# balisujohn/tortoise.cpp

Measured on AMD Instinct MI355X. Metric: audio-seconds/sec end-to-end (AR+diffusion+vocoder), 16 cands x 80 steps, higher is better.
Workload: dtype f16 MFMA inputs / f32 accumulate (diffusion, vocoder convs); f32 weights, f16 KV (AR)

## Files before the change

tortoise.cpp_amd/csrc/api.cpp:

```cpp
#include "common.h"
#include <sched.h>
#include <cctype>
#include <cstddef>
#include <cmath>
#include <algorithm>
#include <chrono>
#include <fstream>
#include <new>

using namespace tts;

hipEvent_t tts::prof_event(tts_ctx *c) {
  if (!c->ev_pool.empty()) { hipEvent_t e = c->ev_pool.back(); c->ev_pool.pop_back(); return e; }
  hipEvent_t e = nullptr;
  (void)hipEventCreate(&e);
  return e;
}

template <class F>
static int guarded(tts_ctx *c, F body) {
  try {
    return body();
  } catch (const std::bad_alloc &) {
    return fail(c, TTS_ERR_LIMIT, "out of host memory");
// ... 130 lines not shown
static void ar_control_store(int which, double value, SamplerParams &sp, int &scope) {
  switch (which) {
  case 0: sp.temp = (float)value; break;
  case 1: sp.top_k = (int)value; break;
  case 2: sp.top_p = (float)value; break;
  case 3: sp.penalty = (float)value; break;
  case 4: scope = (int)value; break;
  case 5: sp.typ_mass = (float)value; break;
  }
}

int tts_set_option(tts_ctx *c, const char *key, double value) {
  if (!c || !key) return TTS_ERR_ARG;
  std::string k(key);
  if (k == "gn_eps") c->gn_eps = (float)value;
  else if (k == "ggml_lut") c->ggml_lut = value != 0;
  else if (k.rfind("prof_only:", 0) == 0) {
    if (value != 0) c->prof_filter.push_back(k.substr(10));
    else c->prof_filter.clear();
  }
  else if (k == "device_topk") c->device_topk = value != 0;
  else if (k == "sampler_threads") {
    if (c->sampler_pool) { sampler_pool_free(c->sampler_pool); c->sampler_pool = nullptr; }
    c->sampler_threads = value < 0 ? -1 : (int)value;
  }
  else if (k == "share_uncond") c->share_uncond = value != 0;
  else if (k == "prof_stride") c->prof_stride = value < 1 ? 1 : (int)value;
  else if (k == "diff_graph") c->diff_graph = value != 0;
  else if (k == "dec_f32_mfma") c->dec_f32_mfma = value != 0;
  else if (k == "attn_f32") c->attn_f32 = value != 0;
  else if (k == "attn_proj_f16") c->attn_proj_f16 = value != 0;
  else if (k == "proj_dual_b") c->proj_dual_b = value != 0;
  else if (k == "gemm_wreg") c->gemm_wreg = value == 1 ? tts_ctx::GEMM_WREG_ALL : value == 2 ? 1 : value == 3 ? 2 : value == 4 ? 4 : 0;
  else if (k == "lc_attn_f32") c->lc_attn_f32 = value != 0;
  else if (k == "latency_mode") c->latency_mode = value != 0;
  else if (k == "fp16_check") c->fp16_check = value != 0;
  else if (k == "rng_fast_normal") c->rng_fast_normal = value != 0;
  else if (k == "noise_pipeline") c->noise_pipeline = value != 0;
  else if (k == "load_device_pack") c->load_device_pack = value != 0;
  else if (k == "load_threads") c->load_threads = value < 0 ? 0 : value > 64 ? 64 : (int)value;
  else if (k == "attn_q64") c->attn_q64 = value < 0 ? 0 : value > 2 ? 2 : (int)value;
  else if (k == "hoist_integrator") c->hoist_integrator = value < 0 ? 0 : (int)value;
  else if (k == "attn_f32_drop") c->attn_f32_drop = (int)value & 7;
  else if (k == "ar_weights") {
    if (value != 0 && value != 1 && value != 2) return fail(c, TTS_ERR_ARG, "ar_weights: 0 (f32), 1 (fp16) or 2 (fp8 e4m3)");
    c->ar_weights = (int)value;
  }
  else if (k == "diff_sampler") {
    if (const char *e = diff_control_error(0, value)) return fail(c, TTS_ERR_ARG, "%s", e);
    c->diff_sampler = (int)value;
  }
  else if (k == "ddim_eta") {
    if (const char *e = diff_control_error(1, value)) return fail(c, TTS_ERR_ARG, "%s", e);
    c->ddim_eta = value;
  }
  else if (k == "cond_free_k") {
    if (const char *e = diff_control_error(2, value)) return fail(c, TTS_ERR_ARG, "%s", e);
    c->cond_free_k = (float)value;
  }
  else if (k == "diff_temperature") {
    if (const char *e = diff_control_error(3, value)) return fail(c, TTS_ERR_ARG, "%s", e);
    c->diff_temperature = value;
  }
  else if (k == "cond_free") {
    if (const char *e = diff_control_error(4, value)) return fail(c, TTS_ERR_ARG, "%s", e);
    c->cond_free = (int)value;
// ... 702 lines not shown
```

tortoise.cpp_amd/csrc/common.h:

```cpp
#pragma once
#include "../../include/tortoise_mi355x.h"
#include <hip/hip_runtime.h>
#include <cstdarg>
#include <cstdint>
#include <cstdio>
#include <cstring>
#include <functional>
#include <map>
#include <memory>
#include <random>
#include <algorithm>
#include <atomic>
#include <condition_variable>
#include <mutex>
#include <new>
#include <string>
#include <thread>
#include <vector>

namespace tts {

struct HostTensor {
  std::vector<float> data;
  int64_t ne[4] = {1, 1, 1, 1};
// ... 90 lines not shown
  std::normal_distribution<double> normal_distribution{0.0, 1.0};
  uint32_t seed_value = 0;
  tts::ArState *ar = nullptr;
  tts::DiffState *diff = nullptr;
  tts::VocState *voc = nullptr;
  tts::ClvpState *clvp = nullptr;
  tts::CvvpState *cvvp = nullptr;
  tts::VoiceEncState *venc = nullptr;
  tts::DiffCondEncState *dcond = nullptr;
  tts::HifiganState *hifigan = nullptr;
  tts::AfeState *afe = nullptr;
  tts::Tokenizer *tok = nullptr;
  tts::ArSession *session = nullptr;
  tts::DiffSession *diff_session = nullptr;
  tts::SamplerPool *sampler_pool = nullptr;
  tts::SamplerParams ar_sp;
  int ar_penalty_scope = 0;
  int device_topk = 1;
  int time_mlp_retries = 0;
  int topk_fallbacks = 0;
  int sampler_threads = -1;
  bool share_uncond = true;
  int rng_shard_offset = 0, rng_shard_total = 0;
  std::vector<int32_t> stop_schedule;
  std::vector<int32_t> ar_stopped;
  bool prof_on = false;
  std::vector<std::string> prof_filter;
  int prof_stride = 1;
  int ar_weights = 0;
  int dec_f32_mfma = 0;
  int attn_f32 = 0;
  static constexpr int GEMM_WREG_ALL = 7;
  int gemm_wreg = GEMM_WREG_ALL;
  int proj_dual_b = 1;
  int attn_f32_drop = 0;
  int lc_attn_f32 = 1;
  int attn_proj_f16 = 0;
  int fp16_check = 0;
  int64_t fp16_bad_weights[2] = {0, 0};
  void *fp16_counts = nullptr;
  int rng_fast_normal = 1;
  int noise_pipeline = 1;
  int load_device_pack = 1;
  int load_threads = 0;
  int attn_q64 = 0;
  int hoist_integrator = 1;
  int latency_mode = 0;
  int diff_sampler = 0;
  double ddim_eta = 0;
  float cond_free_k = 2.0f;
  int cond_free = 1;
  double diff_temperature = 1.0;
  int last_diff_rows = -1, last_diff_seqs = 0;
  bool capturing = false;
  int stream_recaptures = 0;
  int hfg_small_m = 0;
  int diff_graph = 1;
  int prof_eager_every = 8;
  std::map<std::string, tts::ProfEntry> prof;
  std::vector<hipEvent_t> ev_pool;
  hipEvent_t ev0 = nullptr, ev1 = nullptr;
};

namespace tts {

int fail(tts_ctx *ctx, int code, const char *fmt, ...);
// ... 313 lines not shown
```

tortoise.cpp_amd/csrc/diffusion.hip:

```cpp
#include "common.h"
#include "gemm_f16.h"
#include <algorithm>
#include <chrono>
#include <cmath>

namespace tts {

static constexpr int C = 1024, NHEAD = 16, XTC = 128 ;
static constexpr int LAT_MAX_ROWS = 2048;
static constexpr int HOIST_MAX_ROWS = 16384;

__device__ __forceinline__ float silu_dev(float x, int lut) {
  if (lut == 1) {
    float xr = __half2float(__float2half_rn(x));
    return __half2float(__float2half_rn(xr / (1.0f + expf(-xr))));
  }
  if (lut == 2) return x / (1.0f + expf(-x));
  return x * __builtin_amdgcn_rcpf(1.0f + __builtin_amdgcn_exp2f(x * -1.44269504088896f));
}

__global__ __launch_bounds__(256) void gn_stats_kernel(const float *__restrict__ x, const int *__restrict__ seq_start,
                                                       const int *__restrict__ seq_len, float eps, float2 *__restrict__ stats) {
  __shared__ float sh[8];
  const int grp = blockIdx.x, s = blockIdx.y, T = seq_len[s];
// ... 1219 lines not shown
  ProfScope ps(ctx, fam, 2.0 * mv * (n_valid ? n_valid : g.N) * (k_valid ? k_valid : g.nseg * g.kseg));
  TTS_HIP(ctx, launch_gemm_f16(g, ctx->stream));
  if (ctx->fp16_check) {
    if (gemm_mode_qkv(g.mode)) {
      CHECK(fp16_check(ctx, g.outH, (size_t)g.M * g.ldh));
      CHECK(fp16_check(ctx, g.outVt, (size_t)(g.N / 3) * g.ldvt));
    } else if (g.mode == GEMM_OUT_F16) CHECK(fp16_check(ctx, g.outH, (size_t)g.M * g.ldh));
  }
  return TTS_OK;
}

static int gemm_wreg_class(const tts_ctx *ctx, int bit) { return (ctx->gemm_wreg & bit) ? 1 : 0; }
static const __half *gemm_wreg_image(const tts_ctx *ctx, int bit, const Layout &lay, int N, const __half *w, const __half *wf) {
  return gemm_wreg_class(ctx, bit) && gemm_auto_th(lay.rows, N) == 8 ? wf : w;
}

static GemmArgs gemm_base(const Layout &lay, const __half *A, int lda, int nseg, int kseg, const __half *W, int N,
                          const float *bias) {
  GemmArgs g{};
  for (int i = 0; i < 3; i++) { g.A[i] = A; g.row_off[i] = 0; }
  if (nseg == 3) { g.row_off[0] = -1; g.row_off[1] = 0; g.row_off[2] = 1; }
  g.nseg = nseg; g.kseg = kseg; g.lda = lda; g.W = W; g.M = lay.rows; g.N = N; g.bias = bias;
  g.row_seq = lay.d_row_seq.as<int>();
  return g;
}

static int gn_stats(tts_ctx *ctx, const Layout &lay, Work &wk, const float *x) {
  ProfScope ps(ctx, "diff_gn_stats");
  gn_stats_kernel<<<dim3(32, lay.ns), 256, 0, ctx->stream>>>(x, lay.d_start.as<int>(), lay.d_len.as<int>(), ctx->gn_eps,
                                                             wk.stats.as<float2>());
  TTS_HIP(ctx, hipGetLastError());
  return TTS_OK;
}
template <int NT, int NJ>
__global__ __launch_bounds__(NT) void gn_reg_kernel(const float *__restrict__ x, const int *__restrict__ seq_start,
                                                    const int *__restrict__ seq_len, int rows_total, int ns, float eps,
                                                    const float *__restrict__ g, const float *__restrict__ b,
                                                    const float *__restrict__ ss, int do_silu, int lut, __half *__restrict__ y,
                                                    const char *__restrict__ pf0, int pf0_lines, const char *__restrict__ pf1, int pf1_lines,
                                                    const int *__restrict__ seq_step, int ss_step_stride) {
  constexpr int NW = NT / 64, SWEEP = NT / 8;
  __shared__ float sh[2][NW];
  __shared__ unsigned pf_sink[NW][64];
  const int bid = blockIdx.y * 32 + blockIdx.x, nbk = ns * 32, item = (bid & 7) * (nbk >> 3) + (bid >> 3);
  const int s = item >> 5, grp = item & 31;
  const int T = seq_len[s], r0 = seq_start[s];
  const int q = threadIdx.x & 7, c = grp * 32 + q * 4, t0 = threadIdx.x >> 3;
  const float *base = x + (size_t)r0 * C + c;
  float4 v[NJ];
#pragma unroll
  for (int j = 0; j < NJ; j++) {
    const int t = t0 + j * SWEEP;
    v[j] = *(const float4 *)(base + (size_t)min(t, T - 1) * C);
  }
  {
    const int gi = (blockIdx.y * 32 + blockIdx.x) * NT + threadIdx.x, tt = 32 * ns * NT;
    unsigned *sink = &pf_sink[__builtin_amdgcn_readfirstlane(threadIdx.x >> 6)][0];
    for (int l = gi; l < pf0_lines; l += tt) __builtin_amdgcn_global_load_lds((gptr_t)(pf0 + (size_t)l * 128), (lptr_t)sink, 4, 0, 0);
    for (int l = gi; l < pf1_lines; l += tt) __builtin_amdgcn_global_load_lds((gptr_t)(pf1 + (size_t)l * 128), (lptr_t)sink, 4, 0, 0);
  }
  const float4 gg = *(const float4 *)(g + c), bb = *(const float4 *)(b + c);
  float sc4[4] = {1.f, 1.f, 1.f, 1.f}, sh4[4] = {0.f, 0.f, 0.f, 0.f};
  if (ss) {
    if (seq_step) ss += (size_t)seq_step[s] * ss_step_stride;
#pragma unroll
    for (int i = 0; i < 4; i++) { sc4[i] = ss[c + i] + 1.0f; sh4[i] = ss[C + c + i]; }
  }
  float sum = 0.f;
#pragma unroll
  for (int j = 0; j < NJ; j++)
    if (t0 + j * SWEEP < T) sum += (v[j].x + v[j].y) + (v[j].z + v[j].w);
#pragma unroll
  for (int o = 32; o > 0; o >>= 1) sum += __shfl_xor(sum, o);
  if ((threadIdx.x & 63) == 0) sh[0][threadIdx.x >> 6] = sum;
  __syncthreads();
  float tot = 0.f;
#pragma unroll
  for (int w = 0; w < NW; w++) tot += sh[0][w];
  const float n = (float)T * 32.f, mean = tot / n;
  float sq = 0.f;
#pragma unroll
  for (int j = 0; j < NJ; j++) {
    v[j].x -= mean; v[j].y -= mean; v[j].z -= mean; v[j].w -= mean;
    if (t0 + j * SWEEP < T) sq += (v[j].x * v[j].x + v[j].y * v[j].y) + (v[j].z * v[j].z + v[j].w * v[j].w);
  }
#pragma unroll
  for (int o = 32; o > 0; o >>= 1) sq += __shfl_xor(sq, o);
  if ((threadIdx.x & 63) == 0) sh[1][threadIdx.x >> 6] = sq;
  __syncthreads();
  float tsq = 0.f;
#pragma unroll
  for (int w = 0; w < NW; w++) tsq += sh[1][w];
  const float rstd = 1.0f / sqrtf(tsq / n + eps);
  const float ge[4] = {gg.x, gg.y, gg.z, gg.w}, be[4] = {bb.x, bb.y, bb.z, bb.w};
  auto apply = [&](auto mode) {
    constexpr int MODE = decltype(mode)::value;
#pragma unroll
    for (int j = 0; j < NJ; j++) {
      const int t = min(t0 + j * SWEEP, T - 1);
      float e[4] = {v[j].x, v[j].y, v[j].z, v[j].w};
#pragma unroll
      for (int i = 0; i < 4; i++) {
        float u = e[i] * rstd;
        u = u * ge[i];
        u = u + be[i];
        u = u * sc4[i];
        u = u + sh4[i];
        if (MODE) u = silu_dev(u, MODE - 1);
        e[i] = u;
      }
      const __half2 p0 = __floats2half2_rn(e[0], e[1]), p1 = __floats2half2_rn(e[2], e[3]);
      uint2 o;
      o.x = *(const unsigned *)&p0;
      o.y = *(const unsigned *)&p1;
      *(uint2 *)(y + (size_t)(r0 + t) * C + c) = o;
    }
  };
  if (!do_silu) apply(std::integral_constant<int, 0>{});
  else if (lut == 0) apply(std::integral_constant<int, 1>{});
  else if (lut == 1) apply(std::integral_constant<int, 2>{});
  else apply(std::integral_constant<int, 3>{});
  const int gend = (s + 1 < ns) ? seq_start[s + 1] : rows_total;
  for (int r = r0 + T + t0; r < gend; r += SWEEP) *(uint2 *)(y + (size_t)r * C + c) = make_uint2(0u, 0u);
  if (s == 0)
    for (int r = t0; r < r0; r += SWEEP) *(uint2 *)(y + (size_t)r * C + c) = make_uint2(0u, 0u);
  if (pf0_lines | pf1_lines) asm volatile("s_waitcnt vmcnt(0)" ::: "memory");
}

static int gn_fused(tts_ctx *ctx, const Layout &lay, const float *x, const float *g, const float *b, const float *ss, int do_silu,
                    __half *y, const void *wa = nullptr, size_t wa_bytes = 0, const void *wb = nullptr, size_t wb_bytes = 0) {
  ProfScope ps(ctx, "diff_gn_fused");
  if (lay.rows > 4096) { wa_bytes = 0; wb_bytes = 0; }
  const int silu_mode = ctx->ggml_lut ? 1 : ctx->attn_f32 ? 2 : 0;
  auto launch = [&](const int *d_start, int s0, int ns, int row0, int rows, int tmax) {
    const float *xp = x + (size_t)row0 * C;
    __half *yp = y + (size_t)row0 * C;
    const int *d_len = lay.d_len.as<int>() + s0, *step = lay.seq_step_ptr() ? lay.seq_step_ptr() + s0 : nullptr;
#define GN_ARGS xp, d_start, d_len, rows, ns, ctx->gn_eps, g, b, ss, do_silu, silu_mode, yp, \
                (const char *)wa, (int)(wa_bytes >> 7), (const char *)wb, (int)(wb_bytes >> 7), step, lay.ss_step_stride
    if (tmax <= 14 * 64) gn_reg_kernel<512, 14><<<dim3(32, ns), 512, 0, ctx->stream>>>(GN_ARGS);
    else if (tmax <= 18 * 128) gn_reg_kernel<1024, 18><<<dim3(32, ns), 1024, 0, ctx->stream>>>(GN_ARGS);
    else gn_fused_kernel<0><<<dim3(32, ns), 256, 0, ctx->stream>>>(xp, d_start, d_len, rows, ns, ctx->gn_eps, g, b, ss,
                                                                  do_silu, silu_mode, yp, step, lay.ss_step_stride);
#undef GN_ARGS
  };
  if (lay.gn_parts.empty()) launch(lay.d_start.as<int>(), 0, lay.ns, 0, lay.rows, lay.max_len());
  else for (const Layout::GnPart &p : lay.gn_parts) launch(lay.d_start_rel.as<int>() + p.s0, p.s0, p.ns, p.row0, p.rows, p.tmax);
  TTS_HIP(ctx, hipGetLastError());
  return TTS_OK;
}

__global__ __launch_bounds__(256) void gn_apply_kernel(const float *__restrict__ x, const int *__restrict__ chunk_seq, const int *__restrict__ seq_start,
                                                       const int *__restrict__ seq_len, const long long *__restrict__ st, int stripe_ll, float eps, const float *__restrict__ g,
                                                       const float *__restrict__ b, const float *__restrict__ ss, int do_silu, int lut, __half *__restrict__ y,
                                                       const char *__restrict__ pf0, int pf0_lines, const char *__restrict__ pf1, int pf1_lines,
                                                       const int *__restrict__ seq_step, int ss_step_stride) {
  __shared__ float2 mr[32];
  __shared__ unsigned pf_sink[4][64];
  const int r0 = blockIdx.x * 4, s = chunk_seq[blockIdx.x >> 1], c = threadIdx.x * 4;
// ... 134 lines not shown
    }
    TTS_HIP(ctx, hipGetLastError());
  }
  CHECK(fp16_check(ctx, wk.ATT16(), (size_t)lay.rows * C));
  if (f32 && (ctx->attn_f32_drop & 4)) TTS_HIP(ctx, hipMemsetAsync(wk.att16_lo.p, 0, (size_t)(wk.rows + 2) * C * 2, ctx->stream));
  DBG_SUM("attn out", wk.ATT16(), (size_t)lay.rows * C * 2);
  if (f32) {
    GemmArgs p = gemm_base(lay, wk.ATT16(), C, 3, C, w.proj_w_split, C, w.proj_b);
    p.A[0] = wk.ATT16(); p.A[1] = wk.att16_lo.as<__half>() + C; p.A[2] = wk.ATT16();
    p.row_off[0] = p.row_off[1] = p.row_off[2] = 0;
    p.custom_w = 1; p.ldw_ = 2 * C; p.w_off_[0] = 0; p.w_off_[1] = 0; p.w_off_[2] = C;
    p.mode = st_out ? GEMM_OUT_F32_SCALED_STATS : GEMM_OUT_F32_SCALED; p.alpha = w.proj_alpha; p.outF = X; p.ldo = C; p.resid = X;
    p.st_out = st_out; p.st_stripe_ll = (int)st->gn_stripe_ll; p.chunk_seq = lay.d_chunk_seq.as<int>();
    return gemm(ctx, "diff_gemm", p, lay, 0, C);
  }
  if (!ctx->attn_proj_f16) {
    GemmArgs p = gemm_base(lay, wk.ATT16(), C, 2, C, w.proj_w_split, C, w.proj_b);
    p.custom_w = 1; p.ldw_ = 2 * C; p.w_off_[0] = 0; p.w_off_[1] = C;
    p.mode = st_out ? GEMM_OUT_F32_SCALED_STATS : GEMM_OUT_F32_SCALED; p.alpha = w.proj_alpha; p.outF = X; p.ldo = C; p.resid = X;
    p.st_out = st_out; p.st_stripe_ll = (int)st->gn_stripe_ll; p.chunk_seq = lay.d_chunk_seq.as<int>();
    p.dual_b = ctx->proj_dual_b;
    CHECK(gemm(ctx, "diff_gemm", p, lay, 0, C));
    DBG_SUM("attn proj", X, (size_t)lay.rows * C * 4);
    return TTS_OK;
  }
  GemmArgs p = gemm_base(lay, wk.ATT16(), C, 1, C, w.proj_w, C, w.proj_b);
  p.mode = st_out ? GEMM_OUT_F32_STATS : GEMM_OUT_F32; p.outF = X; p.ldo = C; p.resid = X;
  p.st_out = st_out; p.st_stripe_ll = (int)st->gn_stripe_ll; p.chunk_seq = lay.d_chunk_seq.as<int>();
  CHECK(gemm(ctx, "diff_gemm", p, lay));
  DBG_SUM("attn proj", X, (size_t)lay.rows * C * 4);
  return TTS_OK;
}

static int res_block(tts_ctx *ctx, DiffState *st, const Layout &lay, Work &wk, float *X, const ResDev &w, const float *ss,
                     const float *Xin = nullptr, const float *Hpre = nullptr, const long long *st_hpre = nullptr) {
  const float *xin = Xin ? Xin : X;
  const bool lat = st->lat && (Hpre ? st_hpre != nullptr : wk.st_x != nullptr);
  const long long *st_h = st_hpre;
  if (!Hpre) {
    long long *slot = lat ? st->new_stats_slot() : nullptr;
    CHECK(res_in_layers(ctx, st, lay, wk, xin, w, wk.H(), lat ? wk.st_x : nullptr, slot));
    Hpre = wk.H();
    st_h = slot;
  }
  DBG_SUM("res.out ss", ss, (size_t)2 * C * 4);
  DBG_SUM("res.out hpre", Hpre, (size_t)lay.rows * C * 4);
  CHECK(gn(ctx, st, lay, Hpre, lat ? st_h : nullptr, w.out_g, w.out_b, ss, 1, wk.A16(), lat ? w.out_w : gemm_wreg_image(ctx, 4, lay, C, w.out_w, w.out_wf), (size_t)3 * C * C * 2));
  DBG_SUM("res.out gn", wk.A16(), (size_t)lay.rows * C * 2);
  GemmArgs c3 = gemm_base(lay, wk.A16(), C, 3, C, w.out_w, C, w.out_bias);
  c3.Wf = w.out_wf; c3.wreg = gemm_wreg_class(ctx, 4);
  long long *st_out = lat ? st->new_stats_slot() : nullptr;
  c3.mode = st_out ? GEMM_OUT_F32_STATS : GEMM_OUT_F32; c3.outF = X; c3.ldo = C; c3.resid = xin;
  c3.st_out = st_out; c3.st_stripe_ll = (int)st->gn_stripe_ll; c3.chunk_seq = lay.d_chunk_seq.as<int>();
  wk.st_x = st_out;
  CHECK(gemm(ctx, "diff_gemm", c3, lay));
  DBG_SUM("res.out conv", X, (size_t)lay.rows * C * 4);
  return TTS_OK;
}

template <int CTRL> __device__ __forceinline__ float lnk_dpp(float x) {
  return __int_as_float(__builtin_amdgcn_update_dpp(0, __float_as_int(x), CTRL, 0xf, 0xf, false));
}
__device__ __forceinline__ float wave_sum_dpp(float x) {
  auto a = __builtin_amdgcn_permlane32_swap(__float_as_uint(x), __float_as_uint(x), false, false);
  x = __uint_as_float(a[0]) + __uint_as_float(a[1]);
  auto b = __builtin_amdgcn_permlane16_swap(__float_as_uint(x), __float_as_uint(x), false, false);
  x = __uint_as_float(b[0]) + __uint_as_float(b[1]);
  x += lnk_dpp<0x128>(x);
  x += lnk_dpp<0x124>(x);
  x += lnk_dpp<0x122>(x);
  x += lnk_dpp<0x121>(x);
// ... 532 lines not shown
  const auto t_loop = now();
  TTS_HIP(ctx, hipMemcpyAsync(mel_out, r.x.p, total * 4, hipMemcpyDeviceToHost, ctx->stream));
  TTS_HIP(ctx, hipStreamSynchronize(ctx->stream));
  if (timing)
    fprintf(stderr, "[tts timing] diffusion: setup %.1f ms, time MLP + noise %.1f, %d steps %.1f (issued in %.1f, graph capture + instantiate %.1f), mel copy %.1f\n",
            ms(t_begin, r.t_setup), ms(r.t_setup, t_pre), n_steps, ms(t_pre, t_loop), ms(t_pre, t_issued), t_capture, ms(t_loop, now()));
  return TTS_OK;
}
int diff_sample(tts_ctx *ctx, const float *latents, const int32_t *rows, int B, int n_steps, const float *noise, int noise_mode,
                float *mel_out) {
  if (!ctx->diff) return fail(ctx, TTS_ERR_STATE, "diffusion model not loaded");
  if (!latents || !rows || !mel_out || B < 1 || n_steps < 2) return fail(ctx, TTS_ERR_ARG, "tts_diffusion: bad argument");
  for (int c = 0; c < B; c++) if (rows[c] < 1 || rows[c] > 500) return fail(ctx, TTS_ERR_ARG, "latent rows %d out of range", rows[c]);
  return diff_sample_with(ctx, latents, rows, B, nullptr, 0, nullptr, n_steps, noise, noise_mode, mel_out);
}
int diff_sample_voices(tts_ctx *ctx, const float *latents, const int32_t *rows, int B, const float *voice_latents, int n_voices, const int32_t *voice_of,
                       int n_steps, const float *noise, int noise_mode, float *mel_out) {
  if (!ctx->diff) return fail(ctx, TTS_ERR_STATE, "diffusion model not loaded");
  if (!latents || !rows || !mel_out || B < 1 || n_steps < 2 || !voice_latents || !voice_of) return fail(ctx, TTS_ERR_ARG, "tts_diffusion_multi_voice: bad argument");
  if (n_voices < 1 || n_voices > (1 << 20)) return fail(ctx, TTS_ERR_ARG, "tts_diffusion_multi_voice: %d voices", n_voices);
  for (int c = 0; c < B; c++) {
    if (rows[c] < 1 || rows[c] > 500) return fail(ctx, TTS_ERR_ARG, "latent rows %d out of range", rows[c]);
    if (voice_of[c] < 0 || voice_of[c] >= n_voices)
      return fail(ctx, TTS_ERR_ARG, "tts_diffusion_multi_voice: candidate %d names voice %d of %d", c, voice_of[c], n_voices);
  }
  const size_t nf = (size_t)n_voices * 2 * C;
  for (size_t i = 0; i < nf; i++)
    if (!std::isfinite(voice_latents[i])) return fail(ctx, TTS_ERR_ARG, "tts_diffusion_multi_voice: voice %d holds a non-finite value", (int)(i / (2 * C)));
  return diff_sample_with(ctx, latents, rows, B, voice_latents, n_voices, voice_of, n_steps, noise, noise_mode, mel_out);
}

struct PinnedOptions {
  float gn_eps;
  int ggml_lut, attn_f32, attn_proj_f16, proj_dual_b, gemm_wreg, attn_f32_drop, lc_attn_f32, attn_q64, fp16_check, hoist_integrator, diff_graph, latency_mode;
  bool share_uncond;
  static PinnedOptions of(const tts_ctx *c) {
    return PinnedOptions{c->gn_eps, c->ggml_lut, c->attn_f32, c->attn_proj_f16, c->proj_dual_b, c->gemm_wreg, c->attn_f32_drop, c->lc_attn_f32, c->attn_q64,
                         c->fp16_check, c->hoist_integrator, c->diff_graph, c->latency_mode, c->share_uncond};
  }
  void put(tts_ctx *c) const {
    c->gn_eps = gn_eps; c->ggml_lut = ggml_lut; c->attn_f32 = attn_f32; c->attn_proj_f16 = attn_proj_f16; c->proj_dual_b = proj_dual_b; c->gemm_wreg = gemm_wreg;
    c->attn_f32_drop = attn_f32_drop; c->lc_attn_f32 = lc_attn_f32; c->attn_q64 = attn_q64; c->fp16_check = fp16_check; c->hoist_integrator = hoist_integrator;
    c->diff_graph = diff_graph; c->latency_mode = latency_mode; c->share_uncond = share_uncond;
  }
};
struct DiffSession {
  int max_rows = 0, max_req = 0, buf_rows = 0;
  PinnedOptions pinned{};
  int attn_f32 = 0, hoist = 0, graph = 0, sampler = 0;
  bool share_uncond = true, hoisted = false;
  double eta = 0, temperature = 1.0;
  float k = 2.0f;
  int cond_free = 1;
  std::map<int, std::unique_ptr<DiffReq>> reqs;
  std::vector<char> slot_busy;
  int next_id = 0, captures = 0;
  bool dirty = true;
  StepBufs sb;
};
namespace {
struct SessOptions {
  tts_ctx *c;
  PinnedOptions saved;
  SessOptions(tts_ctx *ctx, const DiffSession &s) : c(ctx), saved(PinnedOptions::of(ctx)) { s.pinned.put(ctx); }
  ~SessOptions() { saved.put(c); }
};
}

void diff_session_close(tts_ctx *ctx) {
  if (!ctx->diff_session) return;
  (void)hipStreamSynchronize(ctx->stream);
  delete ctx->diff_session;
  ctx->diff_session = nullptr;
}
int diff_session_captures(const tts_ctx *ctx) { return ctx->diff_session->captures; }
void diff_session_defaults(const tts_ctx *ctx, tts_diff_request *req) {
// ... 197 lines not shown
```

tortoise.cpp_amd/csrc/gemm_f16.h:

```cpp
#pragma once
#include <hip/hip_fp16.h>
#include <hip/hip_runtime.h>
#include <algorithm>
#include <cmath>
#include <cstdlib>
#include <type_traits>

namespace tts {

typedef _Float16 half8 __attribute__((ext_vector_type(8)));
typedef float floatx4 __attribute__((ext_vector_type(4)));

enum { GEMM_OUT_F32 = 0, GEMM_OUT_F16 = 1, GEMM_OUT_QKV = 2, GEMM_OUT_QKV_SPLIT = 3, GEMM_OUT_F32_SCALED = 4, GEMM_OUT_F32_STATS = 5, GEMM_OUT_F32_SCALED_STATS = 6 };
constexpr bool gemm_mode_qkv(int mode) { return mode == GEMM_OUT_QKV || mode == GEMM_OUT_QKV_SPLIT; }
constexpr bool gemm_mode_f32(int mode) { return mode == GEMM_OUT_F32 || mode == GEMM_OUT_F32_SCALED || mode == GEMM_OUT_F32_STATS || mode == GEMM_OUT_F32_SCALED_STATS; }
constexpr bool gemm_mode_scaled(int mode) { return mode == GEMM_OUT_F32_SCALED || mode == GEMM_OUT_F32_SCALED_STATS; }
constexpr bool gemm_mode_stats(int mode) { return mode == GEMM_OUT_F32_STATS || mode == GEMM_OUT_F32_SCALED_STATS; }

struct GemmArgs {
  const __half *A[3];
  int row_off[3];
  int nseg, kseg;
  int lda;
  const __half *W;
// ... 604 lines not shown
      if (t0 + 1 < T) step(t0 + 1, std::integral_constant<int, 1>{});
      if (S == 3 && t0 + 2 < T) step(t0 + 2, std::integral_constant<int, S - 1>{});
    }
  };
  issue(0, std::integral_constant<int, 0>{});
  if (D == 2) issue(1, std::integral_constant<int, 1>{});
#pragma unroll
  for (int i = 0; i < MI; i++)
#pragma unroll
    for (int j = 0; j < 2; j++) asm volatile("" : "+v"(acc[i][j]));
  kloop();
  gemm_epilogue_wreg<MODE, MI, NAT>(g, acc, m0, n0, nblk, wave, fr, fq);
}

static constexpr int GEMM_WREG_D = 1, GEMM_WREG_LDS = (GEMM_WREG_D + 1) * 16384;
template <int MODE, int D = GEMM_WREG_D>
static __global__ __launch_bounds__(256, 4) void gemm_f16_wreg_kernel(GemmArgs g) {
  const int tid = threadIdx.x, lane = tid & 63, wave = __builtin_amdgcn_readfirstlane(tid >> 6);
  int m0, n0, nblk;
  if (!gemm_vh_tile(g, m0, n0, nblk)) return;
  if (gemm_mode_qkv(MODE) && ((n0 + wave * 32) % 192) >= 128) {
    if (nblk > 4) gemm_wreg_body<MODE, 8, D, true>(g, m0, n0, nblk, lane, wave);
    else gemm_wreg_body<MODE, 4, D, true>(g, m0, n0, nblk, lane, wave);
  } else {
    if (nblk > 4) gemm_wreg_body<MODE, 8, D, false>(g, m0, n0, nblk, lane, wave);
    else gemm_wreg_body<MODE, 4, D, false>(g, m0, n0, nblk, lane, wave);
  }
}
static inline bool gemm_takes_wreg(const GemmArgs &g, int th, int ku) {
  return g.wreg > 0 && g.Wf && g.nseg == 1 && !g.custom_w && th == 8 && ku == 1 && (g.kseg >> 6) >= 2 &&
         (g.mode == GEMM_OUT_F32 || g.mode == GEMM_OUT_QKV || g.mode == GEMM_OUT_QKV_SPLIT);
}

static constexpr int CONV3_VH_LDS = (128 + 8) * 128 + 2 * 16384;
template <int MODE, int MI>
__device__ __forceinline__ void gemm_conv3_vh_body(const GemmArgs &g, int m0, int n0, int nblk, int lane, int wave) {
  extern __shared__ __attribute__((aligned(16))) char smem_dyn[];
  char *smem = smem_dyn;
  constexpr int MA = MI > 0 ? MI : 1;
  const int wm = wave >> 1, wn = wave & 1;
  const int my_pa = (2 * nblk + 1 - wave + 3) >> 2;
  const int nchunks = g.kseg >> 6, ldw = 3 * g.kseg, nph = 3 * nchunks;
  const int prow = lane >> 3, pslot = lane & 7;
  const int fr = lane & 15, fq = lane >> 4;
  floatx4 acc[MA][4];
#pragma unroll
  for (int i = 0; i < MI; i++)
#pragma unroll
    for (int j = 0; j < 4; j++) acc[i][j] = (floatx4){0.f, 0.f, 0.f, 0.f};
  char *sa = smem, *sb = smem + (128 + 8) * 128;
  const __half *abase = g.A[0] + (ptrdiff_t)(m0 - 1) * g.lda;
  const __half *wbase = g.W + (size_t)n0 * ldw;
  int aoff[5], boff[4];
#pragma unroll
  for (int i = 0; i < 5; i++) {
    const int row = (wave + 4 * i) * 8 + prow;
    aoff[i] = min(row, g.M - m0 + 1) * g.lda + (pslot ^ lds_swz(row)) * 8;
  }
#pragma unroll
  for (int i = 0; i < 4; i++) {
    const int row = (wave * 4 + i) * 8 + prow;
    boff[i] = row * ldw + (pslot ^ lds_swz(row)) * 8;
  }
  auto stageA = [&](int kc) {
    const __half *src = abase + (min(kc, nchunks - 1) << 6);
#pragma unroll
// ... 328 lines not shown
```

Before: 140.0.

## Fuse res-block input GEMM with following GroupNorm+SiLU via LDS panel kernel

Adds a GEMM kernel in which each block computes a whole sequence's 64-column output panel (up to 896 rows) into LDS, then applies the GroupNorm, scale-shift and SiLU tail directly from that panel to write f16 activations. In the diffusion res_block, when the layout fits and latency stats are off, this replaces the separate f32 GEMM output, stats and gn_reg passes. The aim is to skip the f32 round trip of H through global memory and one or more kernel launches. The cost is large per-block LDS, fewer and longer blocks (one per sequence and column panel), lower occupancy, and padding of short sequences to the fixed panel row count.

```diff
diff --git a/tortoise.cpp_amd/csrc/api.cpp b/tortoise.cpp_amd/csrc/api.cpp
--- a/tortoise.cpp_amd/csrc/api.cpp
+++ b/tortoise.cpp_amd/csrc/api.cpp
@@ -186,6 +186,7 @@
   else if (k == "attn_proj_f16") c->attn_proj_f16 = value != 0;
   else if (k == "proj_dual_b") c->proj_dual_b = value != 0;
   else if (k == "gemm_wreg") c->gemm_wreg = value == 1 ? tts_ctx::GEMM_WREG_ALL : value == 2 ? 1 : value == 3 ? 2 : value == 4 ? 4 : 0;
+  else if (k == "gemm_gn_fuse") c->gemm_gn_fuse = value != 0;
   else if (k == "lc_attn_f32") c->lc_attn_f32 = value != 0;
   else if (k == "latency_mode") c->latency_mode = value != 0;
   else if (k == "fp16_check") c->fp16_check = value != 0;
diff --git a/tortoise.cpp_amd/csrc/common.h b/tortoise.cpp_amd/csrc/common.h
--- a/tortoise.cpp_amd/csrc/common.h
+++ b/tortoise.cpp_amd/csrc/common.h
@@ -146,6 +146,7 @@
   int attn_f32 = 0;
   static constexpr int GEMM_WREG_ALL = 7;
   int gemm_wreg = GEMM_WREG_ALL;
+  int gemm_gn_fuse = 1;
   int proj_dual_b = 1;
   int attn_f32_drop = 0;
   int lc_attn_f32 = 1;
diff --git a/tortoise.cpp_amd/csrc/diffusion.hip b/tortoise.cpp_amd/csrc/diffusion.hip
--- a/tortoise.cpp_amd/csrc/diffusion.hip
+++ b/tortoise.cpp_amd/csrc/diffusion.hip
@@ -1275,33 +1275,20 @@
   TTS_HIP(ctx, hipGetLastError());
   return TTS_OK;
 }
-template <int NT, int NJ>
-__global__ __launch_bounds__(NT) void gn_reg_kernel(const float *__restrict__ x, const int *__restrict__ seq_start,
-                                                    const int *__restrict__ seq_len, int rows_total, int ns, float eps,
-                                                    const float *__restrict__ g, const float *__restrict__ b,
-                                                    const float *__restrict__ ss, int do_silu, int lut, __half *__restrict__ y,
-                                                    const char *__restrict__ pf0, int pf0_lines, const char *__restrict__ pf1, int pf1_lines,
-                                                    const int *__restrict__ seq_step, int ss_step_stride) {
+template <int NT, int NJ, class LOAD, class TOUCH>
+__device__ __forceinline__ void gn_reg_body(LOAD load, TOUCH touch, int s, int c, int T, int r0, const int *__restrict__ seq_start, int rows_total, int ns, float eps,
+                                            const float *__restrict__ g, const float *__restrict__ b, const float *__restrict__ ss, int do_silu, int lut,
+                                            __half *__restrict__ y, const int *__restrict__ seq_step, int ss_step_stride) {
   constexpr int NW = NT / 64, SWEEP = NT / 8;
   __shared__ float sh[2][NW];
-  __shared__ unsigned pf_sink[NW][64];
-  const int bid = blockIdx.y * 32 + blockIdx.x, nbk = ns * 32, item = (bid & 7) * (nbk >> 3) + (bid >> 3);
-  const int s = item >> 5, grp = item & 31;
-  const int T = seq_len[s], r0 = seq_start[s];
-  const int q = threadIdx.x & 7, c = grp * 32 + q * 4, t0 = threadIdx.x >> 3;
-  const float *base = x + (size_t)r0 * C + c;
+  const int t0 = threadIdx.x >> 3;
   float4 v[NJ];
 #pragma unroll
   for (int j = 0; j < NJ; j++) {
     const int t = t0 + j * SWEEP;
-    v[j] = *(const float4 *)(base + (size_t)min(t, T - 1) * C);
-  }
-  {
-    const int gi = (blockIdx.y * 32 + blockIdx.x) * NT + threadIdx.x, tt = 32 * ns * NT;
-    unsigned *sink = &pf_sink[__builtin_amdgcn_readfirstlane(threadIdx.x >> 6)][0];
-    for (int l = gi; l < pf0_lines; l += tt) __builtin_amdgcn_global_load_lds((gptr_t)(pf0 + (size_t)l * 128), (lptr_t)sink, 4, 0, 0);
-    for (int l = gi; l < pf1_lines; l += tt) __builtin_amdgcn_global_load_lds((gptr_t)(pf1 + (size_t)l * 128), (lptr_t)sink, 4, 0, 0);
-  }
+    v[j] = load(min(t, T - 1));
+  }
+  touch();
   const float4 gg = *(const float4 *)(g + c), bb = *(const float4 *)(b + c);
   float sc4[4] = {1.f, 1.f, 1.f, 1.f}, sh4[4] = {0.f, 0.f, 0.f, 0.f};
   if (ss) {
@@ -1367,7 +1354,44 @@
   for (int r = r0 + T + t0; r < gend; r += SWEEP) *(uint2 *)(y + (size_t)r * C + c) = make_uint2(0u, 0u);
   if (s == 0)
     for (int r = t0; r < r0; r += SWEEP) *(uint2 *)(y + (size_t)r * C + c) = make_uint2(0u, 0u);
+}
+template <int NT, int NJ>
+__global__ __launch_bounds__(NT) void gn_reg_kernel(const float *__restrict__ x, const int *__restrict__ seq_start,
+                                                    const int *__restrict__ seq_len, int rows_total, int ns, float eps,
+                                                    const float *__restrict__ g, const float *__restrict__ b,
+                                                    const float *__restrict__ ss, int do_silu, int lut, __half *__restrict__ y,
+                                                    const char *__restrict__ pf0, int pf0_lines, const char *__restrict__ pf1, int pf1_lines,
+                                                    const int *__restrict__ seq_step, int ss_step_stride) {
+  constexpr int NW = NT / 64;
+  __shared__ unsigned pf_sink[NW][64];
+  const int bid = blockIdx.y * 32 + blockIdx.x, nbk = ns * 32, item = (bid & 7) * (nbk >> 3) + (bid >> 3);
+  const int s = item >> 5, grp = item & 31;
+  const int T = seq_len[s], r0 = seq_start[s];
+  const int q = threadIdx.x & 7, c = grp * 32 + q * 4;
+  const float *base = x + (size_t)r0 * C + c;
+  auto touch = [&]() {
+    const int gi = (blockIdx.y * 32 + blockIdx.x) * NT + threadIdx.x, tt = 32 * ns * NT;
+    unsigned *sink = &pf_sink[__builtin_amdgcn_readfirstlane(threadIdx.x >> 6)][0];
+    for (int l = gi; l < pf0_lines; l += tt) __builtin_amdgcn_global_load_lds((gptr_t)(pf0 + (size_t)l * 128), (lptr_t)sink, 4, 0, 0);
+    for (int l = gi; l < pf1_lines; l += tt) __builtin_amdgcn_global_load_lds((gptr_t)(pf1 + (size_t)l * 128), (lptr_t)sink, 4, 0, 0);
+  };
+  gn_reg_body<NT, NJ>([&](int t) { return *(const float4 *)(base + (size_t)t * C); }, touch, s, c, T, r0, seq_start, rows_total, ns, eps, g, b, ss, do_silu, lut, y, seq_step,
+                      ss_step_stride);
   if (pf0_lines | pf1_lines) asm volatile("s_waitcnt vmcnt(0)" ::: "memory");
+}
+struct GnPanelTail {
+  __device__ __forceinline__ void operator()(const GemmGnPanelArgs &a, int s, int T, int r0, int c0, const char *panel) const {
+    const int q = threadIdx.x & 7;
+    gn_reg_body<512, 14>([&](int t) { return *(const float4 *)(panel + gnp_panel_f4(t, q)); }, []() {}, s, c0 + q * 4, T, r0, a.seq_start, a.rows_total, a.ns, a.eps, a.gn_g,
+                         a.gn_b, a.ss, a.do_silu, a.lut, a.y, a.seq_step, a.ss_step_stride);
+  }
+};
+
+static inline hipError_t launch_gemm_gn_panel(const GemmGnPanelArgs &a, hipStream_t s) {
+  static bool raised = false;
+  if (!raised) { (void)hipFuncSetAttribute((const void *)gemm_f16_gn_panel_kernel<GnPanelTail>, hipFuncAttributeMaxDynamicSharedMemorySize, GEMM_GN_PANEL_LDS); raised = true; }
+  gemm_f16_gn_panel_kernel<GnPanelTail><<<gemm_gn_panel_grid(a.ns, a.N), 512, GEMM_GN_PANEL_LDS, s>>>(a, GnPanelTail{});
+  return hipGetLastError();
 }
 
 static int gn_fused(tts_ctx *ctx, const Layout &lay, const float *x, const float *g, const float *b, const float *ss, int do_silu,
@@ -1568,11 +1592,40 @@
   return TTS_OK;
 }
 
+static int gemm_gn_panel(tts_ctx *ctx, const Layout &lay, const __half *A, const __half *Wf, const float *bias, const float *g, const float *b, const float *ss, __half *y) {
+  double mv = 0;
+  for (int l : lay.len) mv += l;
+  {
+    ProfScope ps(ctx, "diff_gemm_k1", 2.0 * mv * C * C);
+    GemmGnPanelArgs a{};
+    a.A = A; a.lda = C; a.Wf = Wf; a.N = C; a.K = C; a.bias = bias;
+    a.seq_start = lay.d_start.as<int>(); a.seq_len = lay.d_len.as<int>(); a.ns = lay.ns; a.rows_total = lay.rows;
+    a.eps = ctx->gn_eps; a.gn_g = g; a.gn_b = b; a.ss = ss; a.do_silu = 1; a.lut = ctx->ggml_lut ? 1 : ctx->attn_f32 ? 2 : 0;
+    a.y = y; a.seq_step = lay.seq_step_ptr(); a.ss_step_stride = lay.ss_step_stride;
+    TTS_HIP(ctx, launch_gemm_gn_panel(a, ctx->stream));
+  }
+  return fp16_check(ctx, y, (size_t)lay.rows * C);
+}
+
 static int res_block(tts_ctx *ctx, DiffState *st, const Layout &lay, Work &wk, float *X, const ResDev &w, const float *ss,
                      const float *Xin = nullptr, const float *Hpre = nullptr, const long long *st_hpre = nullptr) {
   const float *xin = Xin ? Xin : X;
   const bool lat = st->lat && (Hpre ? st_hpre != nullptr : wk.st_x != nullptr);
   const long long *st_h = st_hpre;
+#ifdef TTS_DEBUG_CHECKSUM
+  constexpr bool debug_sums = true;
+#else
+  constexpr bool debug_sums = false;
+#endif
+  if (!Hpre && gemm_gn_panel_takes(ctx->gemm_gn_fuse, st->lat, debug_sums, w.in_wf != nullptr, lay.gn_parts.empty() ? lay.max_len() : GEMM_GN_PANEL_ROWS + 1, lay.rows, C, C)) {
+    CHECK(gn(ctx, st, lay, xin, nullptr, w.in_g, w.in_b, nullptr, 1, wk.A16()));
+    CHECK(gemm_gn_panel(ctx, lay, wk.A16(), w.in_wf, w.in_bias, w.out_g, w.out_b, ss, wk.ATT16()));
+    GemmArgs c3 = gemm_base(lay, wk.ATT16(), C, 3, C, w.out_w, C, w.out_bias);
+    c3.Wf = w.out_wf; c3.wreg = gemm_wreg_class(ctx, 4);
+    c3.mode = GEMM_OUT_F32; c3.outF = X; c3.ldo = C; c3.resid = xin;
+    wk.st_x = nullptr;
+    return gemm(ctx, "diff_gemm", c3, lay);
+  }
   if (!Hpre) {
     long long *slot = lat ? st->new_stats_slot() : nullptr;
     CHECK(res_in_layers(ctx, st, lay, wk, xin, w, wk.H(), lat ? wk.st_x : nullptr, slot));
@@ -2171,16 +2224,16 @@
 
 struct PinnedOptions {
   float gn_eps;
-  int ggml_lut, attn_f32, attn_proj_f16, proj_dual_b, gemm_wreg, attn_f32_drop, lc_attn_f32, attn_q64, fp16_check, hoist_integrator, diff_graph, latency_mode;
+  int ggml_lut, attn_f32, attn_proj_f16, proj_dual_b, gemm_wreg, attn_f32_drop, lc_attn_f32, attn_q64, fp16_check, hoist_integrator, diff_graph, latency_mode, gemm_gn_fuse;
   bool share_uncond;
   static PinnedOptions of(const tts_ctx *c) {
     return PinnedOptions{c->gn_eps, c->ggml_lut, c->attn_f32, c->attn_proj_f16, c->proj_dual_b, c->gemm_wreg, c->attn_f32_drop, c->lc_attn_f32, c->attn_q64,
-                         c->fp16_check, c->hoist_integrator, c->diff_graph, c->latency_mode, c->share_uncond};
+                         c->fp16_check, c->hoist_integrator, c->diff_graph, c->latency_mode, c->gemm_gn_fuse, c->share_uncond};
   }
   void put(tts_ctx *c) const {
     c->gn_eps = gn_eps; c->ggml_lut = ggml_lut; c->attn_f32 = attn_f32; c->attn_proj_f16 = attn_proj_f16; c->proj_dual_b = proj_dual_b; c->gemm_wreg = gemm_wreg;
     c->attn_f32_drop = attn_f32_drop; c->lc_attn_f32 = lc_attn_f32; c->attn_q64 = attn_q64; c->fp16_check = fp16_check; c->hoist_integrator = hoist_integrator;
-    c->diff_graph = diff_graph; c->latency_mode = latency_mode; c->share_uncond = share_uncond;
+    c->diff_graph = diff_graph; c->latency_mode = latency_mode; c->gemm_gn_fuse = gemm_gn_fuse; c->share_uncond = share_uncond;
   }
 };
 struct DiffSession {
diff --git a/tortoise.cpp_amd/csrc/gemm_f16.h b/tortoise.cpp_amd/csrc/gemm_f16.h
--- a/tortoise.cpp_amd/csrc/gemm_f16.h
+++ b/tortoise.cpp_amd/csrc/gemm_f16.h
@@ -660,6 +660,147 @@
          (g.mode == GEMM_OUT_F32 || g.mode == GEMM_OUT_QKV || g.mode == GEMM_OUT_QKV_SPLIT);
 }
 
+struct GemmGnPanelArgs {
+  const __half *A; int lda;
+  const __half *Wf;
+  int N, K;
+  const float *bias;
+  const int *seq_start, *seq_len; int ns, rows_total;
+  float eps; const float *gn_g, *gn_b, *ss; int do_silu, lut; __half *y; const int *seq_step; int ss_step_stride;
+};
+static constexpr int GEMM_GN_PANEL_ROWS = 896, GEMM_GN_PANEL_LDS = GEMM_GN_PANEL_ROWS * 128;
+__device__ __forceinline__ int gnp_panel_f4(int t, int q) { return t * 128 + ((q ^ (t & 7)) << 4); }
+template <int OFF> __device__ __forceinline__ void gnp_lds_read(half8 &d, unsigned addr) {
+  asm volatile("ds_read_b128 %0, %1 offset:%2" : "=v"(d) : "v"(addr), "i"(OFF));
+}
+static inline int gemm_auto_th(int M, int N);
+static inline bool gemm_gn_panel_takes(int option, bool stats, bool debug_sums, bool has_wf, int max_len, int rows, int N, int K) {
+  return option != 0 && !stats && !debug_sums && has_wf && max_len >= 1 && max_len <= GEMM_GN_PANEL_ROWS && gemm_auto_th(rows, N) == 8 && (N % 64) == 0 && K >= 64 && (K % 64) == 0;
+}
+static inline int gemm_gn_panel_grid(int ns, int N) { return 8 * ((ns * (N >> 6) + 7) / 8); }
+
+template <class TAIL>
+static __global__ __launch_bounds__(512) void gemm_f16_gn_panel_kernel(GemmGnPanelArgs a, TAIL tail) {
+  extern __shared__ __attribute__((aligned(16))) char smem_dyn[];
+  char *smem = smem_dyn;
+  const int tid = threadIdx.x, lane = tid & 63, wave = __builtin_amdgcn_readfirstlane(tid >> 6);
+  const int np = a.N >> 6, nitems = a.ns * np, xcd = blockIdx.x & 7, idx = blockIdx.x >> 3;
+  const int i0 = (int)((long long)nitems * xcd >> 3), i1 = (int)((long long)nitems * (xcd + 1) >> 3);
+  if (idx >= i1 - i0) return;
+  const int item = i0 + idx, s = item / np, n0 = (item - s * np) << 6;
+  const int T = a.seq_len[s], r0 = a.seq_start[s];
+  const int KT = a.K >> 6, fr = lane & 15, fq = lane >> 4;
+  const int rb = wave * 8 + (lane >> 3), lda2 = a.lda * 2;
+  const unsigned coloff = (unsigned)(((lane & 7) ^ lds_swz(lane >> 3)) << 4);
+  const char *aseg = (const char *)(a.A + (size_t)r0 * a.lda);
+  const size_t wstride = (size_t)(a.K >> 5) * 512;
+  const __half *wp0 = a.Wf + (size_t)(n0 >> 4) * wstride, *wp1 = wp0 + wstride, *wp2 = wp1 + wstride, *wp3 = wp2 + wstride;
+  const unsigned wlane = lane * 16;
+  const unsigned lds0 = (unsigned)(size_t)(lptr_t)smem + wave * 7 * 2048;
+  const unsigned fb0 = lds0 + lds_off(fr, fq), fb1 = lds0 + lds_off(fr, 4 + fq);
+  floatx4 acc[7][4];
+#pragma unroll
+  for (int i = 0; i < 7; i++)
+#pragma unroll
+    for (int j = 0; j < 4; j++) acc[i][j] = (floatx4){0.f, 0.f, 0.f, 0.f};
+  half8 w[2][4];
+  auto dma = [&](int t) {
+    const char *ab = aseg + (t << 7);
+    int rbv = rb;
+    asm volatile("" : "+v"(rbv));
+#pragma unroll
+    for (int i = 0; i < 14; i++) {
+      const unsigned off = (unsigned)(min(rbv + 64 * i, T - 1) * lda2) + coloff;
+      __builtin_amdgcn_global_load_lds((gptr_t)(ab + off), (lptr_t)(smem + (wave + 8 * i) * 1024), 16, 0, 0);
+    }
+  };
+  auto wload = [&](int t, auto ks_c) {
+    constexpr int KS = decltype(ks_c)::value;
+    const size_t o = (size_t)t * 1024;
+    wreg_load<KS * 1024>(w[KS][0], wp0 + o, wlane);
+    wreg_load<KS * 1024>(w[KS][1], wp1 + o, wlane);
+    wreg_load<KS * 1024>(w[KS][2], wp2 + o, wlane);
+    wreg_load<KS * 1024>(w[KS][3], wp3 + o, wlane);
+  };
+  auto pin_acc = [&]() {
+#pragma unroll
+    for (int j = 0; j < 4; j++)
+      asm volatile("" : "+v"(acc[0][j]), "+v"(acc[1][j]), "+v"(acc[2][j]), "+v"(acc[3][j]), "+v"(acc[4][j]), "+v"(acc[5][j]), "+v"(acc[6][j]));
+  };
+  auto step = [&](int t, auto last_c) {
+    constexpr bool LAST = decltype(last_c)::value;
+    wreg_wait<4>(w[0][0], w[0][1], w[0][2], w[0][3]);
+    __builtin_amdgcn_s_barrier();
+    asm volatile("" ::: "memory");
+    half8 af[2][7];
+    gnp_lds_read<0 * 2048>(af[0][0], fb0);
+    gnp_lds_read<1 * 2048>(af[0][1], fb0);
+    gnp_lds_read<2 * 2048>(af[0][2], fb0);
+    gnp_lds_read<3 * 2048>(af[0][3], fb0);
+    gnp_lds_read<4 * 2048>(af[0][4], fb0);
+    gnp_lds_read<5 * 2048>(af[0][5], fb0);
+    gnp_lds_read<6 * 2048>(af[0][6], fb0);
+    gnp_lds_read<0 * 2048>(af[1][0], fb1);
+    gnp_lds_read<1 * 2048>(af[1][1], fb1);
+    gnp_lds_read<2 * 2048>(af[1][2], fb1);
+    gnp_lds_read<3 * 2048>(af[1][3], fb1);
+    gnp_lds_read<4 * 2048>(af[1][4], fb1);
+    gnp_lds_read<5 * 2048>(af[1][5], fb1);
+    gnp_lds_read<6 * 2048>(af[1][6], fb1);
+    asm volatile("s_waitcnt lgkmcnt(0)"
+                 : "+v"(af[0][0]), "+v"(af[0][1]), "+v"(af[0][2]), "+v"(af[0][3]), "+v"(af[0][4]), "+v"(af[0][5]), "+v"(af[0][6]), "+v"(af[1][0]), "+v"(af[1][1]),
+                   "+v"(af[1][2]), "+v"(af[1][3]), "+v"(af[1][4]), "+v"(af[1][5]), "+v"(af[1][6])
+                 :
+                 : "memory");
+    __builtin_amdgcn_s_barrier();
+    asm volatile("" ::: "memory");
+    if (!LAST) dma(t + 1);
+#pragma unroll
+    for (int i = 0; i < 7; i++)
+#pragma unroll
+      for (int j = 0; j < 4; j++) acc[i][j] = __builtin_amdgcn_mfma_f32_16x16x32_f16(w[0][j], af[0][i], acc[i][j], 0, 0, 0);
+    if (!LAST) {
+      pin_acc();
+      wload(t + 1, std::integral_constant<int, 0>{});
+    }
+    wreg_wait<LAST ? 0 : 18>(w[1][0], w[1][1], w[1][2], w[1][3]);
+#pragma unroll
+    for (int i = 0; i < 7; i++)
+#pragma unroll
+      for (int j = 0; j < 4; j++) acc[i][j] = __builtin_amdgcn_mfma_f32_16x16x32_f16(w[1][j], af[1][i], acc[i][j], 0, 0, 0);
+    if (!LAST) {
+      pin_acc();
+      wload(t + 1, std::integral_constant<int, 1>{});
+    }
+  };
+  dma(0);
+  wload(0, std::integral_constant<int, 0>{});
+  wload(0, std::integral_constant<int, 1>{});
+  for (int t = 0; t + 1 < KT; t++) step(t, std::false_type{});
+  step(KT - 1, std::true_type{});
+  const bool hb = a.bias != nullptr;
+  const float *bp = hb ? a.bias : (const float *)a.Wf;
+  float4 b4[4];
+#pragma unroll
+  for (int j = 0; j < 4; j++) b4[j] = *(const float4 *)(bp + n0 + j * 16 + fq * 4);
+#pragma unroll
+  for (int j = 0; j < 4; j++) b4[j] = hb ? b4[j] : make_float4(0.f, 0.f, 0.f, 0.f);
+#pragma unroll
+  for (int gi = 0; gi < 2; gi++) {
+#pragma unroll
+    for (int i = 0; i < 7; i++) {
+      const int row = (wave * 7 + i) * 16 + fr;
+#pragma unroll
+      for (int jj = 0; jj < 2; jj++) {
+        const int j = gi * 2 + jj;
+        *(float4 *)(smem + gnp_panel_f4(row, jj * 4 + fq)) = make_float4(acc[i][j][0] + b4[j].x, acc[i][j][1] + b4[j].y, acc[i][j][2] + b4[j].z, acc[i][j][3] + b4[j].w);
+      }
+    }
+    __syncthreads();
+    tail(a, s, T, r0, n0 + gi * 32, smem);
+  }
+}
+
 static constexpr int CONV3_VH_LDS = (128 + 8) * 128 + 2 * 16384;
 template <int MODE, int MI>
 __device__ __forceinline__ void gemm_conv3_vh_body(const GemmArgs &g, int m0, int n0, int nblk, int lane, int wave) {
diff --git a/tortoise.cpp_amd/testlib/gemm_gn_panel_harness.hip b/tortoise.cpp_amd/testlib/gemm_gn_panel_harness.hip
--- /dev/null
+++ b/tortoise.cpp_amd/testlib/gemm_gn_panel_harness.hip
@@ -0,0 +1,147 @@
+#include "../csrc/diffusion.hip"
+
+#include <cstdint>
+#include <cstring>
+#include <vector>
+
+using namespace tts;
+hipEvent_t tts::prof_event(tts_ctx *) { return nullptr; }
+
+extern "C" {
+
+enum { TTS_GNP_TEST_MARGIN = 4096, TTS_GNP_TEST_SENTINEL = 0xCB, TTS_GNP_TEST_MAX_SEQ = 64, TTS_GNP_TEST_MAX_ROWS = 8192, TTS_GNP_TEST_MAX_TABLE = 64,
+       TTS_GNP_TEST_MAX_STRIDE = 1 << 16 };
+
+struct tts_gnp_case {
+  int ns, rows, N, K;
+  int do_silu, lut, n_steps, ss_step_stride;
+  float eps;
+  const int *start, *len, *seq_step;
+  const uint16_t *A, *W;
+  const float *bias, *g, *b, *ss;
+  void *out_pair, *out_fused;
+};
+
+int tts_gnp_test_margin(void) { return TTS_GNP_TEST_MARGIN; }
+int tts_gnp_test_takes(int option, int stats, int debug_sums, int has_wf, int max_len, int rows, int N, int K) {
+  return gemm_gn_panel_takes(option, stats != 0, debug_sums != 0, has_wf != 0, max_len, rows, N, K) ? 1 : 0;
+}
+int tts_gnp_test_grid(int ns, int N) { return gemm_gn_panel_grid(ns, N); }
+int tts_gnp_test_lds(void) { return GEMM_GN_PANEL_LDS; }
+
+}
+
+namespace {
+
+struct Dev {
+  char *p = nullptr;
+  size_t bytes = 0;
+  ~Dev() { if (p) (void)hipFree(p); }
+  hipError_t alloc(size_t payload, int fill) {
+    bytes = payload;
+    hipError_t e = hipMalloc((void **)&p, payload + 2 * TTS_GNP_TEST_MARGIN);
+    if (e != hipSuccess) { p = nullptr; return e; }
+    return hipMemset(p, fill, payload + 2 * TTS_GNP_TEST_MARGIN);
+  }
+  char *data() const { return p ? p + TTS_GNP_TEST_MARGIN : nullptr; }
+  hipError_t put(const void *h) { return hipMemcpy(data(), h, bytes, hipMemcpyHostToDevice); }
+  hipError_t get_all(void *h) const { return hipMemcpy(h, p, bytes + 2 * TTS_GNP_TEST_MARGIN, hipMemcpyDeviceToHost); }
+};
+
+int nw_of(int N) { return (N + 127) / 128 * 128; }
+
+bool valid(const tts_gnp_case &c) {
+  if (!c.A || !c.W || !c.g || !c.b || !c.out_pair || !c.out_fused || !c.start || !c.len) return false;
+  if (c.rows < 128 || c.rows % 128 || c.rows > TTS_GNP_TEST_MAX_ROWS) return false;
+  if (c.N < 64 || c.N % 64 || c.N > C || c.K < 128 || c.K % 64 || c.K > 2048) return false;
+  if (c.ns < 1 || c.ns > TTS_GNP_TEST_MAX_SEQ) return false;
+  long long prev_end = 0;
+  for (int s = 0; s < c.ns; s++) {
+    const long long st = c.start[s], ln = c.len[s];
+    if (st < prev_end || st % 8 || ln < 1 || ln > GEMM_GN_PANEL_ROWS || st + ln + 1 > c.rows) return false;
+    prev_end = st + ln + 1;
+  }
+  if (c.lut < 0 || c.lut > 2 || (c.do_silu != 0 && c.do_silu != 1)) return false;
+  if (c.seq_step && !c.ss) return false;
+  if (c.ss) {
+    if (c.n_steps < 1 || c.n_steps > TTS_GNP_TEST_MAX_TABLE || c.ss_step_stride < 0 || c.ss_step_stride > TTS_GNP_TEST_MAX_STRIDE) return false;
+    if (!c.seq_step && c.n_steps != 1) return false;
+    if (c.seq_step)
+      for (int s = 0; s < c.ns; s++)
+        if (c.seq_step[s] < 0 || c.seq_step[s] >= c.n_steps) return false;
+  }
+  return true;
+}
+
+}
+
+extern "C" {
+
+int tts_gnp_test_validate(const tts_gnp_case *c) { return c && valid(*c) ? 0 : (int)hipErrorInvalidValue; }
+
+#define HT(x) do { hipError_t e_ = (x); if (e_ != hipSuccess) return (int)e_; } while (0)
+
+int tts_gnp_test_run(const tts_gnp_case *cp) {
+  if (!cp || !valid(*cp)) return (int)hipErrorInvalidValue;
+  const tts_gnp_case &c = *cp;
+  const int rows = c.rows, Nw = nw_of(c.N), K = c.K;
+  GemmArgs g{};
+  for (int i = 0; i < 3; i++) { g.A[i] = nullptr; g.row_off[i] = 0; }
+  g.nseg = 1; g.kseg = K; g.lda = K; g.M = rows; g.N = Nw; g.mode = GEMM_OUT_F32; g.ldo = C; g.wreg = 1; g.th = 8;
+  g.Wf = (const __half *)c.W;
+  if (gemm_plan(g).err != hipSuccess || gemm_plan(g).kernel != GEMM_KERNEL_WREG) return (int)hipErrorInvalidValue;
+
+  std::vector<uint16_t> wf((size_t)Nw * K);
+  for (int n = 0; n < Nw; n++)
+    for (int k = 0; k < K; k++) wf[gemm_wfrag_index(n, k, K)] = c.W[(size_t)n * K + k];
+  std::vector<int> rs(rows, -1);
+  for (int s = 0; s < c.ns; s++)
+    for (int t = 0; t < c.len[s]; t++) rs[c.start[s] + t] = s;
+
+  Dev A, W, Wf, bias, gg, bb, ss, step, start, len, rseq, H, yp, yf;
+  HT(A.alloc((size_t)rows * K * 2, 0)); HT(A.put(c.A));
+  HT(W.alloc((size_t)Nw * K * 2, 0)); HT(W.put(c.W));
+  HT(Wf.alloc((size_t)Nw * K * 2, 0)); HT(Wf.put(wf.data()));
+  if (c.bias) { HT(bias.alloc((size_t)Nw * 4, 0)); HT(bias.put(c.bias)); }
+  HT(gg.alloc((size_t)C * 4, 0)); HT(gg.put(c.g));
+  HT(bb.alloc((size_t)C * 4, 0)); HT(bb.put(c.b));
+  if (c.ss) {
+    HT(ss.alloc(((size_t)(c.n_steps - 1) * c.ss_step_stride + 2 * C) * 4, 0)); HT(ss.put(c.ss));
+    if (c.seq_step) { HT(step.alloc((size_t)c.ns * 4, 0)); HT(step.put(c.seq_step)); }
+  }
+  HT(start.alloc((size_t)c.ns * 4, 0)); HT(start.put(c.start));
+  HT(len.alloc((size_t)c.ns * 4, 0)); HT(len.put(c.len));
+  HT(rseq.alloc((size_t)rows * 4, 0)); HT(rseq.put(rs.data()));
+  HT(H.alloc((size_t)rows * C * 4, 0));
+  HT(yp.alloc((size_t)rows * C * 2, TTS_GNP_TEST_SENTINEL));
+  HT(yf.alloc((size_t)rows * C * 2, TTS_GNP_TEST_SENTINEL));
+
+  for (int i = 0; i < 3; i++) g.A[i] = (const __half *)A.data();
+  g.W = (const __half *)W.data(); g.Wf = (const __half *)Wf.data(); g.bias = (const float *)bias.data();
+  g.row_seq = (const int *)rseq.data(); g.outF = (float *)H.data(); g.resid = nullptr;
+  const int *d_start = (const int *)start.data(), *d_len = (const int *)len.data(), *d_step = (const int *)step.data();
+  GemmGnPanelArgs a{};
+  a.A = (const __half *)A.data(); a.lda = K; a.Wf = (const __half *)Wf.data(); a.N = c.N; a.K = K; a.bias = (const float *)bias.data();
+  a.seq_start = d_start; a.seq_len = d_len; a.ns = c.ns; a.rows_total = rows;
+  a.eps = c.eps; a.gn_g = (const float *)gg.data(); a.gn_b = (const float *)bb.data(); a.ss = (const float *)ss.data(); a.do_silu = c.do_silu; a.lut = c.lut;
+  a.y = (__half *)yf.data(); a.seq_step = d_step; a.ss_step_stride = c.ss_step_stride;
+
+  hipStream_t s;
+  HT(hipStreamCreateWithFlags(&s, hipStreamNonBlocking));
+  hipError_t e = hipDeviceSynchronize();
+  if (e == hipSuccess) e = launch_gemm_f16(g, s);
+  if (e == hipSuccess) {
+    gn_reg_kernel<512, 14><<<dim3(32, c.ns), 512, 0, s>>>((const float *)H.data(), d_start, d_len, rows, c.ns, c.eps, a.gn_g, a.gn_b, a.ss, c.do_silu, c.lut,
+                                                          (__half *)yp.data(), nullptr, 0, nullptr, 0, d_step, c.ss_step_stride);
+    e = hipGetLastError();
+  }
+  if (e == hipSuccess) e = launch_gemm_gn_panel(a, s);
+  const hipError_t es = hipStreamSynchronize(s);
+  (void)hipStreamDestroy(s);
+  if (e != hipSuccess || es != hipSuccess) return (int)(e != hipSuccess ? e : es);
+  HT(yp.get_all(c.out_pair));
+  HT(yf.get_all(c.out_fused));
+  return 0;
+}
+
+}
```

Result: faster. 142.9, median of 6 (+2.1%).
